# saidwivedi/TokenHMR

Hardware: AMD Instinct MI355X
Metric: crops_per_sec (higher is better)
Workload: dtype f32 (fp32 in / accumulate / out; the ViT GEMMs multiply each fp32 operand as three bf16 pieces on the bf16 MFMA pipe, six products per pair: `vit_gemm` split3; the fp32-MFMA mode is `exact_f32_mode`); 1 GPU; TokenHMR full path (ViT-H/16 + 6-layer token decoder + VQ lookup/decode + SMPL LBS), 256x256 crops, random-init weights; batch_per_gpu=64, global_batch=64, vit_depth=32, parallelism=dp1, allgather_outputs=False, vit_gemm=split3, ranks=1

## Files before the change

tokenhmr_amd/csrc/attention_b16.hip:

```cpp
#include "common.h"
#include "attention_device.h"
#include "gemm_split_device.h"

namespace {

constexpr int KB = 64;
constexpr int NBLK = NTOK / KB;
constexpr int KRS = 224;
constexpr int VRS = 160;
constexpr int KPL = KB * KRS;
constexpr int VPL = HD * VRS;
constexpr int K_IMG = 3 * KPL, V_IMG = 3 * VPL;
static_assert(2 * (K_IMG + V_IMG) <= 160 * 1024, "two workgroups per CU");
static_assert(V_IMG >= 4 * 16 * 480, "the split3 epilogue assembles 4 waves x 16 rows x 480 bytes in the dead V^T image");
constexpr float LOG2E_F = 1.44269504088896340736f;

typedef uint32_t u32x2v __attribute__((ext_vector_type(2)));

__device__ __forceinline__ bf16x8 pieces8(uint32_t a, uint32_t b, uint32_t c, uint32_t d) {
    return __builtin_bit_cast(bf16x8, u32x4{a, b, c, d});
}

template <int QT, bool SPLIT, int ABL = 0, int EARLY = 0, int OCC = 2>
__global__ __launch_bounds__(256, OCC) void vit_attention_b16_kernel(const float* __restrict__ qkv, float* __restrict__ out, int nitems) {
    constexpr int QB = 3 / QT;
    static_assert(QT == 1 || QT == 3, "192 queries = QB workgroups x 4 waves x QT tiles of 16");
    __shared__ __attribute__((aligned(16))) char smem[K_IMG + V_IMG];
    char* const kimg = smem;
    char* const vimg = smem + K_IMG;
    const int tid = threadIdx.x, lane = tid & 63;
    const int wave = __builtin_amdgcn_readfirstlane(tid >> 6);
    const int l15 = lane & 15, g = lane >> 4;
    const int xcd = blockIdx.x & 7, within = blockIdx.x >> 3, wpx = gridDim.x >> 3, per_xcd = nitems >> 3;
    int it = within;
    if (it >= per_xcd) return;
    struct Item { int crop, hcol, q0; };
    auto item_of = [&](int i) {
        const int lg = xcd * per_xcd + i, bh = lg / QB, qb = lg - bh * QB;
        return Item{bh / NH, (bh % NH) * HD, (qb * 4 + wave) * 16 * QT};
    };
    auto rsrc_of = [&](int crop) { return __builtin_amdgcn_make_buffer_rsrc(const_cast<float*>(qkv + (int64_t)crop * NTOK * QKV_LD), 0, NTOK * QKV_LD * 4, 0x00020000); };
    auto ld4 = [&](const Item& im, int uoff_floats, uint32_t off) {
        const u32x4 r = __builtin_amdgcn_raw_buffer_load_b128(rsrc_of(im.crop), off, uoff_floats * 4, 0);
        return f32x4{__uint_as_float(r[0]), __uint_as_float(r[1]), __uint_as_float(r[2]), __uint_as_float(r[3])};
    };
    auto ld1 = [&](const Item& im, int uoff_floats, uint32_t off) { return __uint_as_float(__builtin_amdgcn_raw_buffer_load_b32(rsrc_of(im.crop), off, uoff_floats * 4, 0)); };

    const int kkey = tid >> 2, kpart = tid & 3;
    const int vdg = (tid & 7) + 8 * ((tid >> 4) & 1), vkq = ((tid >> 5) & 3) | (((tid >> 3) & 1) << 2) | ((tid >> 7) << 3);
    const uint32_t koff = (uint32_t)(kkey * QKV_LD + kpart * 4) * 4u;
    const uint32_t voff = (uint32_t)(vkq * 4 * QKV_LD + vdg) * 4u;
    const uint32_t qoff = (uint32_t)(l15 * QKV_LD + g * 8) * 4u;
    char* const kdst = kimg + kkey * KRS + kpart * 8;
    char* const vdst = vimg + vdg * VRS + (((4 * (vkq >> 3) + (vkq & 3)) ^ ((vdg >> 2) & 1)) * 16) + 8 * ((vkq >> 2) & 1);
    f32x4 kr[5];
    float vr[5][4];
    auto load_k = [&](const Item& im, int blk) {
        const int ub = im.hcol + DIM + blk * KB * QKV_LD;
#pragma unroll
        for (int m = 0; m < 5; ++m) kr[m] = ld4(im, ub + m * 16, koff);
    };
    auto write_k = [&]() {
#pragma unroll
        for (int m = 0; m < 5; ++m) {
            uint32_t H[2], M[2], L[2];
            split3_pair(kr[m][0], kr[m][1], H[0], M[0], L[0]);
            split3_pair(kr[m][2], kr[m][3], H[1], M[1], L[1]);
            char* o = kdst + m * 32;
            *reinterpret_cast<u32x2v*>(o) = u32x2v{H[0], H[1]};
            *reinterpret_cast<u32x2v*>(o + KPL) = u32x2v{M[0], M[1]};
            *reinterpret_cast<u32x2v*>(o + 2 * KPL) = u32x2v{L[0], L[1]};
        }
    };
    auto load_v = [&](const Item& im, int blk) {
        const int ub = im.hcol + 2 * DIM + blk * KB * QKV_LD;
#pragma unroll
        for (int m = 0; m < 5; ++m)
#pragma unroll
            for (int r = 0; r < 4; ++r) vr[m][r] = ld1(im, ub + r * QKV_LD + m * 16, voff);
    };
    auto write_v = [&]() {
#pragma unroll
        for (int m = 0; m < 5; ++m) {
            uint32_t H[2], M[2], L[2];
            split3_pair(vr[m][0], vr[m][1], H[0], M[0], L[0]);
            split3_pair(vr[m][2], vr[m][3], H[1], M[1], L[1]);
            char* o = vdst + m * 16 * VRS;
            *reinterpret_cast<u32x2v*>(o) = u32x2v{H[0], H[1]};
            *reinterpret_cast<u32x2v*>(o + VPL) = u32x2v{M[0], M[1]};
            *reinterpret_cast<u32x2v*>(o + 2 * VPL) = u32x2v{L[0], L[1]};
        }
    };

    f32x4 qraw[QT][2];
    auto load_q = [&](const Item& im, int s) {
#pragma unroll
        for (int qt = 0; qt < QT; ++qt) {
            const int ub = im.hcol + (im.q0 + qt * 16) * QKV_LD + s * 32;
            if (s < 2 || g < 2) {
                qraw[qt][0] = ld4(im, ub, qoff);
                qraw[qt][1] = ld4(im, ub + 4, qoff);
            } else {
                qraw[qt][0] = f32x4{0.f, 0.f, 0.f, 0.f};
                qraw[qt][1] = f32x4{0.f, 0.f, 0.f, 0.f};
            }
        }
    };
    bf16x8 qf[QT][3];
    auto split_q = [&]() {
#pragma unroll
        for (int qt = 0; qt < QT; ++qt) {
            uint32_t H[4], M[4], L[4];
            split3_pair(qraw[qt][0][0], qraw[qt][0][1], H[0], M[0], L[0]);
            split3_pair(qraw[qt][0][2], qraw[qt][0][3], H[1], M[1], L[1]);
            split3_pair(qraw[qt][1][0], qraw[qt][1][1], H[2], M[2], L[2]);
            split3_pair(qraw[qt][1][2], qraw[qt][1][3], H[3], M[3], L[3]);
            qf[qt][0] = pieces8(H[0], H[1], H[2], H[3]);
            qf[qt][1] = pieces8(M[0], M[1], M[2], M[3]);
            qf[qt][2] = pieces8(L[0], L[1], L[2], L[3]);
        }
    };

    const char* const kfr = kimg + l15 * KRS + g * 16;
    const char* const vfr = vimg + l15 * VRS + ((g ^ ((l15 >> 2) & 1)) * 16);

    Item cur = item_of(it);
    load_k(cur, 0);
    load_q(cur, 0);
    for (int idx = tid; idx < 3 * KB * 2; idx += 256) {
        const int pl = idx / (2 * KB), rem = idx - pl * (2 * KB);
        *reinterpret_cast<u32x4*>(kimg + pl * KPL + (rem >> 1) * KRS + 160 + (rem & 1) * 16) = u32x4{0u, 0u, 0u, 0u};
    }
    write_k();
    __syncthreads();

#pragma unroll 1
    for (;;) {
        const bool has_next = it + wpx < per_xcd;
        const Item nxt = has_next ? item_of(it + wpx) : cur;
        f32x4 o[QT][5];
        float lsum[QT], cneg[QT];
#pragma unroll
        for (int qt = 0; qt < QT; ++qt) {
#pragma unroll
            for (int dt = 0; dt < 5; ++dt) o[qt][dt] = f32x4{0.f, 0.f, 0.f, 0.f};
            lsum[qt] = 0.f;
            cneg[qt] = 3.0e38f;
        }
#pragma unroll 1
        for (int blk = 0; blk < NBLK; ++blk) {
            const bool more = blk + 1 < NBLK;
            f32x4 s[QT][4];
#pragma unroll
            for (int qt = 0; qt < QT; ++qt)
#pragma unroll
                for (int kt = 0; kt < 4; ++kt) s[qt][kt] = f32x4{0.f, 0.f, 0.f, 0.f};
            bf16x8 kc[3], kn[3];
#pragma unroll
            for (int pc = 0; pc < 3; ++pc) kc[pc] = *reinterpret_cast<const bf16x8*>(kfr + pc * KPL);
#pragma unroll
            for (int st = 0; st < 3; ++st) {
                if constexpr (EARLY > 0 && (ABL & 2) == 0) {
                    if (st == EARLY - 1) {
                        load_v(cur, blk);
                        if (more) load_k(cur, blk + 1);
                        else if (has_next) load_k(nxt, 0);
                    }
                }
                if ((ABL & 4) == 0 || blk == 0) split_q();
                if (st + 1 < 3 && ((ABL & 1) == 0 || blk == 0)) load_q(cur, st + 1);
#pragma unroll
                for (int kt = 0; kt < 4; ++kt) {
                    const int nx = st * 4 + kt + 1;
                    if (nx < 12) {
#pragma unroll
                        for (int pc = 0; pc < 3; ++pc)
                            kn[pc] = *reinterpret_cast<const bf16x8*>(kfr + pc * KPL + (nx % 4) * 16 * KRS + (nx / 4) * 64);
                    }
                    __builtin_amdgcn_sched_barrier(0);
#pragma unroll
                    for (int p = 0; p < NPROD; ++p)
#pragma unroll
                        for (int qt = 0; qt < QT; ++qt)
                            s[qt][kt] = __builtin_amdgcn_mfma_f32_16x16x32_bf16(kc[piece_w(p)], qf[qt][piece_a(p)], s[qt][kt], 0, 0, 0);
                    __builtin_amdgcn_sched_barrier(0);
#pragma unroll
                    for (int pc = 0; pc < 3; ++pc) kc[pc] = kn[pc];
                }
            }
            if constexpr ((ABL & 2) == 0) {
                if constexpr (EARLY == 0) {
                    load_v(cur, blk);
                    if (more) load_k(cur, blk + 1);
                    else if (has_next) load_k(nxt, 0);
                }
            } else {
#pragma unroll
                for (int m = 0; m < 5; ++m) {
                    kr[m] = s[0][m & 3];
                    asm volatile("" : "+v"(kr[m]));
#pragma unroll
                    for (int r = 0; r < 4; ++r) {
                        vr[m][r] = s[0][(m + r) & 3][r];
                        asm volatile("" : "+v"(vr[m][r]));
                    }
                }
            }
            __syncthreads();
#pragma unroll
            for (int qt = 0; qt < QT; ++qt) {
                float m = s[qt][0][0];
#pragma unroll
                for (int kt = 0; kt < 4; ++kt)
#pragma unroll
                    for (int r = 0; r < 4; ++r) m = fmaxf(m, s[qt][kt][r]);
                m = fmaxf(m, __shfl_xor(m, 16, 64));
                m = fmaxf(m, __shfl_xor(m, 32, 64));
                const float c = fminf(-(m * LOG2E_F), cneg[qt]);
                const float alpha = __builtin_amdgcn_exp2f(c - cneg[qt]);
                cneg[qt] = c;
                lsum[qt] *= alpha;
#pragma unroll
                for (int dt = 0; dt < 5; ++dt) o[qt][dt] = o[qt][dt] * alpha;
                const f32x2 c2 = splat2(c), l2 = splat2(LOG2E_F);
                f32x2 sum2 = splat2(0.f);
#pragma unroll
                for (int kt = 0; kt < 4; ++kt)
#pragma unroll
                    for (int hh = 0; hh < 2; ++hh) {
                        const f32x2 t = __builtin_elementwise_fma(f32x2{s[qt][kt][2 * hh], s[qt][kt][2 * hh + 1]}, l2, c2);
                        const f32x2 e = f32x2{__builtin_amdgcn_exp2f(t.x), __builtin_amdgcn_exp2f(t.y)};
                        s[qt][kt][2 * hh] = e.x;
                        s[qt][kt][2 * hh + 1] = e.y;
                        sum2 += e;
                    }
                lsum[qt] += sum2.x + sum2.y;
            }
            write_v();
            if (more || has_next) write_k();
            __syncthreads();
            if constexpr ((ABL & 1) == 0) {
                if (more) load_q(cur, 0);
                else if (has_next) load_q(nxt, 0);
            } else if (!more && has_next) load_q(nxt, 0);
            bf16x8 vc[3], vn[3];
#pragma unroll
            for (int pc = 0; pc < 3; ++pc) vc[pc] = *reinterpret_cast<const bf16x8*>(vfr + pc * VPL);
#pragma unroll
            for (int st = 0; st < 2; ++st) {
                bf16x8 pf[QT][3];
#pragma unroll
                for (int qt = 0; qt < QT; ++qt) {
                    uint32_t H[4], M[4], L[4];
                    split3_pair(s[qt][2 * st][0], s[qt][2 * st][1], H[0], M[0], L[0]);
                    split3_pair(s[qt][2 * st][2], s[qt][2 * st][3], H[1], M[1], L[1]);
                    split3_pair(s[qt][2 * st + 1][0], s[qt][2 * st + 1][1], H[2], M[2], L[2]);
                    split3_pair(s[qt][2 * st + 1][2], s[qt][2 * st + 1][3], H[3], M[3], L[3]);
                    pf[qt][0] = pieces8(H[0], H[1], H[2], H[3]);
                    pf[qt][1] = pieces8(M[0], M[1], M[2], M[3]);
                    pf[qt][2] = pieces8(L[0], L[1], L[2], L[3]);
                }
#pragma unroll
                for (int dt = 0; dt < 5; ++dt) {
                    const int nx = st * 5 + dt + 1;
                    if (nx < 10) {
#pragma unroll
                        for (int pc = 0; pc < 3; ++pc)
                            vn[pc] = *reinterpret_cast<const bf16x8*>(vfr + pc * VPL + (nx % 5) * 16 * VRS + (nx / 5) * 64);
                    }
                    __builtin_amdgcn_sched_barrier(0);
#pragma unroll
                    for (int p = 0; p < NPROD; ++p)
#pragma unroll
                        for (int qt = 0; qt < QT; ++qt)
                            o[qt][dt] = __builtin_amdgcn_mfma_f32_16x16x32_bf16(vc[piece_w(p)], pf[qt][piece_a(p)], o[qt][dt], 0, 0, 0);
                    __builtin_amdgcn_sched_barrier(0);
#pragma unroll
                    for (int pc = 0; pc < 3; ++pc) vc[pc] = vn[pc];
                }
            }
        }

        float inv[QT];
#pragma unroll
        for (int qt = 0; qt < QT; ++qt) {
            float l = lsum[qt];
            l += __shfl_xor(l, 16, 64);
            l += __shfl_xor(l, 32, 64);
            inv[qt] = 1.0f / l;
        }
        if constexpr (SPLIT) {
            __syncthreads();
            char* const stg = vimg + wave * (16 * 480);
            char* const orow = reinterpret_cast<char*>(out) + ((int64_t)cur.crop * NTOK + cur.q0) * (DIM * 6) + cur.hcol * 6;
#pragma unroll
            for (int qt = 0; qt < QT; ++qt) {
                char* const srow = stg + l15 * 480;
#pragma unroll
                for (int pr = 0; pr < 2; ++pr) {
                    f32x4 x = o[qt][2 * pr] * inv[qt], y = o[qt][2 * pr + 1] * inv[qt];
#pragma unroll
                    for (int j = 0; j < 4; ++j) {
                        typedef uint32_t u32x2_t __attribute__((ext_vector_type(2)));
                        const u32x2_t sw = __builtin_amdgcn_permlane16_swap(__float_as_uint(x[j]), __float_as_uint(y[j]), false, false);
                        x[j] = __uint_as_float(sw.x);
                        y[j] = __uint_as_float(sw.y);
                    }
                    uint32_t H[4], M[4], L[4];
                    split3_pair(x[0], x[1], H[0], M[0], L[0]);
                    split3_pair(x[2], x[3], H[1], M[1], L[1]);
                    split3_pair(y[0], y[1], H[2], M[2], L[2]);
                    split3_pair(y[2], y[3], H[3], M[3], L[3]);
                    char* c = srow + ((2 * pr + (g & 1)) * 2 + (g >> 1)) * 48;
                    *reinterpret_cast<u32x4*>(c) = u32x4{H[0], H[1], H[2], H[3]};
                    *reinterpret_cast<u32x4*>(c + 16) = u32x4{M[0], M[1], M[2], M[3]};
                    *reinterpret_cast<u32x4*>(c + 32) = u32x4{L[0], L[1], L[2], L[3]};
                }
                {
                    const f32x4 v = o[qt][4] * inv[qt];
                    uint32_t H[2], M[2], L[2];
                    split3_pair(v[0], v[1], H[0], M[0], L[0]);
                    split3_pair(v[2], v[3], H[1], M[1], L[1]);
                    char* c = srow + (8 + (g >> 1)) * 48 + (g & 1) * 8;
                    *reinterpret_cast<u32x2v*>(c) = u32x2v{H[0], H[1]};
                    *reinterpret_cast<u32x2v*>(c + 16) = u32x2v{M[0], M[1]};
                    *reinterpret_cast<u32x2v*>(c + 32) = u32x2v{L[0], L[1]};
                }
#pragma unroll
                for (int i = 0; i < 8; ++i) {
                    const int c = i * 64 + lane;
                    if (i < 7 || lane < 32) {
                        const u32x4 v = *reinterpret_cast<const u32x4*>(stg + c * 16);
                        const int r = c / 30;
                        *reinterpret_cast<u32x4*>(orow + (int64_t)(qt * 16 + r) * (DIM * 6) + (c - r * 30) * 16) = v;
                    }
                }
            }
        } else {
            float* obase = out + (int64_t)cur.crop * NTOK * DIM + cur.hcol;
#pragma unroll
            for (int qt = 0; qt < QT; ++qt)
#pragma unroll
                for (int dt = 0; dt < 5; ++dt)
                    *reinterpret_cast<f32x4*>(obase + (int64_t)(cur.q0 + qt * 16 + l15) * DIM + dt * 16 + g * 4) = o[qt][dt] * inv[qt];
        }
        if (!has_next) break;
        cur = nxt;
        it += wpx;
    }
}

}

int launch_vit_attention_b16(const float* qkv, void* out, int B, bool out_split, int qt, hipStream_t s) {
    if (B <= 0 || (qt != 0 && qt != 1 && qt != 3)) return -1;
    if (qt == 0) qt = B <= 20 ? 1 : 3;
    float* o = reinterpret_cast<float*>(out);
    const int nitems = B * NH * (3 / qt);
    static_assert(NH % 8 == 0, "items per crop must divide by the XCD count");
    dim3 grid(nitems < 512 ? nitems : 512);
#ifdef THMR_EXPERIMENTS
    {
        const char* gk = thmr_knob("THMR_ATTN_GRID");
        const int gcap = gk ? atoi(gk) : 0;
        if (gcap >= 8 && (gcap % 8) == 0 && (unsigned)gcap < grid.x) grid = dim3(gcap);
        const char* ek = thmr_knob("THMR_ATTN_EARLY");
        const int early = ek ? atoi(ek) : 0;
        const char* ok = thmr_knob("THMR_ATTN_OCC");
        if (ok && ok[0] == '1' && qt == 3 && out_split) {
            if (grid.x > 256) grid = dim3(256);
            switch (early) {
                case 0: hipLaunchKernelGGL((vit_attention_b16_kernel<3, true, 0, 0, 1>), grid, dim3(256), 0, s, qkv, o, nitems); break;
                case 1: hipLaunchKernelGGL((vit_attention_b16_kernel<3, true, 0, 1, 1>), grid, dim3(256), 0, s, qkv, o, nitems); break;
                case 2: hipLaunchKernelGGL((vit_attention_b16_kernel<3, true, 0, 2, 1>), grid, dim3(256), 0, s, qkv, o, nitems); break;
                case 3: hipLaunchKernelGGL((vit_attention_b16_kernel<3, true, 0, 3, 1>), grid, dim3(256), 0, s, qkv, o, nitems); break;
                default: return -1;
            }
            return hipGetLastError() == hipSuccess ? 0 : -2;
        }
        if (early > 0 && qt == 3 && out_split) {
            switch (early) {
                case 1: hipLaunchKernelGGL((vit_attention_b16_kernel<3, true, 0, 1>), grid, dim3(256), 0, s, qkv, o, nitems); break;
                case 2: hipLaunchKernelGGL((vit_attention_b16_kernel<3, true, 0, 2>), grid, dim3(256), 0, s, qkv, o, nitems); break;
                case 3: hipLaunchKernelGGL((vit_attention_b16_kernel<3, true, 0, 3>), grid, dim3(256), 0, s, qkv, o, nitems); break;
                default: return -1;
            }
            return hipGetLastError() == hipSuccess ? 0 : -2;
        }
        const char* k = thmr_knob("THMR_ATTN_ABL");
        const int abl = k ? atoi(k) : 0;
        if (abl > 0 && qt == 3 && out_split) {
            switch (abl) {
                case 1: hipLaunchKernelGGL((vit_attention_b16_kernel<3, true, 1>), grid, dim3(256), 0, s, qkv, o, nitems); break;
                case 2: hipLaunchKernelGGL((vit_attention_b16_kernel<3, true, 2>), grid, dim3(256), 0, s, qkv, o, nitems); break;
                case 3: hipLaunchKernelGGL((vit_attention_b16_kernel<3, true, 3>), grid, dim3(256), 0, s, qkv, o, nitems); break;
                case 4: hipLaunchKernelGGL((vit_attention_b16_kernel<3, true, 4>), grid, dim3(256), 0, s, qkv, o, nitems); break;
                case 5: hipLaunchKernelGGL((vit_attention_b16_kernel<3, true, 5>), grid, dim3(256), 0, s, qkv, o, nitems); break;
                case 7: hipLaunchKernelGGL((vit_attention_b16_kernel<3, true, 7>), grid, dim3(256), 0, s, qkv, o, nitems); break;
                default: return -1;
            }
            return hipGetLastError() == hipSuccess ? 0 : -2;
        }
    }
#endif
    if (qt == 1) {
        if (out_split) hipLaunchKernelGGL((vit_attention_b16_kernel<1, true>), grid, dim3(256), 0, s, qkv, o, nitems);
        else hipLaunchKernelGGL((vit_attention_b16_kernel<1, false>), grid, dim3(256), 0, s, qkv, o, nitems);
    } else {
        if (out_split) hipLaunchKernelGGL((vit_attention_b16_kernel<3, true>), grid, dim3(256), 0, s, qkv, o, nitems);
        else hipLaunchKernelGGL((vit_attention_b16_kernel<3, false>), grid, dim3(256), 0, s, qkv, o, nitems);
    }
    return hipGetLastError() == hipSuccess ? 0 : -2;
}
```

Measured before the change: 855.9 crops/s.

## Keep Q pieces resident across key blocks and interleave softmax with attention MFMAs

Adds a RES mode that loads and splits all three Q slices once per item and keeps them in registers, so the per-block Q reload and re-split go away. Adds TILE modes that interleave one query tile's softmax and P splitting with the next tile's QK/PV MFMAs using sched_group_barrier placement. For B>=32 the default switches to resident Q with early K/V requests and occupancy 1 (grid capped at 256). This trades more registers and lower occupancy for less repeated work and better overlap.

```diff
diff --git a/tokenhmr_amd/csrc/attention_b16.hip b/tokenhmr_amd/csrc/attention_b16.hip
--- a/tokenhmr_amd/csrc/attention_b16.hip
+++ b/tokenhmr_amd/csrc/attention_b16.hip
@@ -21,10 +21,12 @@
     return __builtin_bit_cast(bf16x8, u32x4{a, b, c, d});
 }
 
-template <int QT, bool SPLIT, int ABL = 0, int EARLY = 0, int OCC = 2>
+template <int QT, bool SPLIT, int RES = 0, int EARLY = 0, int OCC = 2, int VPG = 2>
 __global__ __launch_bounds__(256, OCC) void vit_attention_b16_kernel(const float* __restrict__ qkv, float* __restrict__ out, int nitems) {
     constexpr int QB = 3 / QT;
     static_assert(QT == 1 || QT == 3, "192 queries = QB workgroups x 4 waves x QT tiles of 16");
+    constexpr bool TILE = RES == 2 || RES == 3;
+    static_assert(!TILE || QT == 3, "the per-tile interleave needs a wave with more than one query tile");
     __shared__ __attribute__((aligned(16))) char smem[K_IMG + V_IMG];
     char* const kimg = smem;
     char* const vimg = smem + K_IMG;
@@ -92,33 +94,38 @@
         }
     };
 
-    f32x4 qraw[QT][2];
-    auto load_q = [&](const Item& im, int s) {
+    constexpr int QS = RES ? 3 : 1;
+    f32x4 qraw[QS][QT][2];
+    auto load_q = [&](const Item& im, int s, int slot) {
 #pragma unroll
         for (int qt = 0; qt < QT; ++qt) {
             const int ub = im.hcol + (im.q0 + qt * 16) * QKV_LD + s * 32;
             if (s < 2 || g < 2) {
-                qraw[qt][0] = ld4(im, ub, qoff);
-                qraw[qt][1] = ld4(im, ub + 4, qoff);
+                qraw[slot][qt][0] = ld4(im, ub, qoff);
+                qraw[slot][qt][1] = ld4(im, ub + 4, qoff);
             } else {
-                qraw[qt][0] = f32x4{0.f, 0.f, 0.f, 0.f};
-                qraw[qt][1] = f32x4{0.f, 0.f, 0.f, 0.f};
-            }
-        }
-    };
-    bf16x8 qf[QT][3];
-    auto split_q = [&]() {
+                qraw[slot][qt][0] = f32x4{0.f, 0.f, 0.f, 0.f};
+                qraw[slot][qt][1] = f32x4{0.f, 0.f, 0.f, 0.f};
+            }
+        }
+    };
+    bf16x8 qf[QS][QT][3];
+    auto split_q = [&](int slot) {
 #pragma unroll
         for (int qt = 0; qt < QT; ++qt) {
             uint32_t H[4], M[4], L[4];
-            split3_pair(qraw[qt][0][0], qraw[qt][0][1], H[0], M[0], L[0]);
-            split3_pair(qraw[qt][0][2], qraw[qt][0][3], H[1], M[1], L[1]);
-            split3_pair(qraw[qt][1][0], qraw[qt][1][1], H[2], M[2], L[2]);
-            split3_pair(qraw[qt][1][2], qraw[qt][1][3], H[3], M[3], L[3]);
-            qf[qt][0] = pieces8(H[0], H[1], H[2], H[3]);
-            qf[qt][1] = pieces8(M[0], M[1], M[2], M[3]);
-            qf[qt][2] = pieces8(L[0], L[1], L[2], L[3]);
-        }
+            split3_pair(qraw[slot][qt][0][0], qraw[slot][qt][0][1], H[0], M[0], L[0]);
+            split3_pair(qraw[slot][qt][0][2], qraw[slot][qt][0][3], H[1], M[1], L[1]);
+            split3_pair(qraw[slot][qt][1][0], qraw[slot][qt][1][1], H[2], M[2], L[2]);
+            split3_pair(qraw[slot][qt][1][2], qraw[slot][qt][1][3], H[3], M[3], L[3]);
+            qf[slot][qt][0] = pieces8(H[0], H[1], H[2], H[3]);
+            qf[slot][qt][1] = pieces8(M[0], M[1], M[2], M[3]);
+            qf[slot][qt][2] = pieces8(L[0], L[1], L[2], L[3]);
+        }
+    };
+    auto load_q_item = [&](const Item& im) {
+#pragma unroll
+        for (int s = 0; s < 3; ++s) load_q(im, s, s);
     };
 
     const char* const kfr = kimg + l15 * KRS + g * 16;
@@ -126,7 +133,8 @@
 
     Item cur = item_of(it);
     load_k(cur, 0);
-    load_q(cur, 0);
+    if constexpr (RES) load_q_item(cur);
+    else load_q(cur, 0, 0);
     for (int idx = tid; idx < 3 * KB * 2; idx += 256) {
         const int pl = idx / (2 * KB), rem = idx - pl * (2 * KB);
         *reinterpret_cast<u32x4*>(kimg + pl * KPL + (rem >> 1) * KRS + 160 + (rem & 1) * 16) = u32x4{0u, 0u, 0u, 0u};
@@ -147,136 +155,255 @@
             lsum[qt] = 0.f;
             cneg[qt] = 3.0e38f;
         }
+        f32x4 s[QT][4];
+        float smax[QT], salpha[QT], sum0[QT], sum1[QT];
+        auto pin = [](auto&... v) {
+            if constexpr (RES >= 2) (..., [](auto& x) { asm volatile("" : "+v"(x)); }(v));
+        };
+        auto softmax_part = [&](int qt, int part) {
+            if (part == 0) {
+                float m = s[qt][0][0];
+#pragma unroll
+                for (int kt = 0; kt < 2; ++kt)
+#pragma unroll
+                    for (int r = 0; r < 4; ++r) m = fmaxf(m, s[qt][kt][r]);
+                smax[qt] = m;
+                pin(smax[qt]);
+            } else if (part == 1) {
+                float m = smax[qt];
+#pragma unroll
+                for (int kt = 2; kt < 4; ++kt)
+#pragma unroll
+                    for (int r = 0; r < 4; ++r) m = fmaxf(m, s[qt][kt][r]);
+                smax[qt] = m;
+                pin(smax[qt]);
+            } else if (part == 2) {
+                float m = smax[qt];
+                m = fmaxf(m, __shfl_xor(m, 16, 64));
+                m = fmaxf(m, __shfl_xor(m, 32, 64));
+                const float c = fminf(-(m * LOG2E_F), cneg[qt]);
+                salpha[qt] = __builtin_amdgcn_exp2f(c - cneg[qt]);
+                cneg[qt] = c;
+                sum0[qt] = 0.f;
+                sum1[qt] = 0.f;
+                pin(salpha[qt], cneg[qt]);
+            } else if (part == 3) {
+#pragma unroll
+                for (int dt = 0; dt < 5; ++dt)
+#pragma unroll
+                    for (int r = 0; r < 4; ++r) {
+                        o[qt][dt][r] = o[qt][dt][r] * salpha[qt];
+                        if constexpr (RES == 3) {
+                            if (r & 1) asm volatile("" : "+v"(o[qt][dt]));
+                        }
+                    }
+                pin(o[qt][0], o[qt][1], o[qt][2], o[qt][3], o[qt][4]);
+            } else {
+                const int kt = (part - 4) >> 1, hh = (part - 4) & 1;
+                const float e0 = __builtin_amdgcn_exp2f(__builtin_fmaf(s[qt][kt][2 * hh], LOG2E_F, cneg[qt]));
+                const float e1 = __builtin_amdgcn_exp2f(__builtin_fmaf(s[qt][kt][2 * hh + 1], LOG2E_F, cneg[qt]));
+                s[qt][kt][2 * hh] = e0;
+                s[qt][kt][2 * hh + 1] = e1;
+                sum0[qt] += e0;
+                sum1[qt] += e1;
+                if (part == 11) lsum[qt] = __builtin_fmaf(lsum[qt], salpha[qt], sum0[qt] + sum1[qt]);
+                pin(s[qt][kt], sum0[qt], sum1[qt], lsum[qt]);
+            }
+        };
+        uint32_t pw[QT][2][3][4];
+        auto psplit_part = [&](int qt, int part) {
+            const int st = part >> 2, j = part & 3;
+            const float x0 = s[qt][2 * st + (j >> 1)][2 * (j & 1)], x1 = s[qt][2 * st + (j >> 1)][2 * (j & 1) + 1];
+            if constexpr (RES == 3) {
+#pragma clang fp contract(off)
+                const uint32_t H = cvt_pk_bf16(x0, x1);
+                float r0 = x0 - __uint_as_float(H << 16), r1 = x1 - __uint_as_float(H & 0xffff0000u);
+                asm volatile("" : "+v"(r0));
+                const uint32_t M = cvt_pk_bf16(r0, r1);
+                r0 = r0 - __uint_as_float(M << 16);
+                asm volatile("" : "+v"(r0));
+                r1 = r1 - __uint_as_float(M & 0xffff0000u);
+                pw[qt][st][0][j] = H;
+                pw[qt][st][1][j] = M;
+                pw[qt][st][2][j] = cvt_pk_bf16(r0, r1);
+            } else split3_pair(x0, x1, pw[qt][st][0][j], pw[qt][st][1][j], pw[qt][st][2][j]);
+            pin(pw[qt][st][0][j], pw[qt][st][1][j], pw[qt][st][2][j]);
+        };
+        auto pfrag = [&](int qt, int st, int pc) { return pieces8(pw[qt][st][pc][0], pw[qt][st][pc][1], pw[qt][st][pc][2], pw[qt][st][pc][3]); };
+        auto place = [&]() {
+#pragma unroll
+            for (int p = 0; p < NPROD; ++p) {
+                __builtin_amdgcn_sched_group_barrier(0x8, 1, 0);
+                __builtin_amdgcn_sched_group_barrier(0x2, VPG, 0);
+            }
+        };
 #pragma unroll 1
         for (int blk = 0; blk < NBLK; ++blk) {
             const bool more = blk + 1 < NBLK;
-            f32x4 s[QT][4];
-#pragma unroll
-            for (int qt = 0; qt < QT; ++qt)
-#pragma unroll
-                for (int kt = 0; kt < 4; ++kt) s[qt][kt] = f32x4{0.f, 0.f, 0.f, 0.f};
+            auto request_kv = [&]() {
+                load_v(cur, blk);
+                if (more) load_k(cur, blk + 1);
+                else if (has_next) load_k(nxt, 0);
+            };
+            if constexpr (RES) {
+                if (blk == 0) {
+#pragma unroll
+                    for (int st = 0; st < 3; ++st) split_q(st);
+                }
+            }
             bf16x8 kc[3], kn[3];
 #pragma unroll
             for (int pc = 0; pc < 3; ++pc) kc[pc] = *reinterpret_cast<const bf16x8*>(kfr + pc * KPL);
-#pragma unroll
-            for (int st = 0; st < 3; ++st) {
-                if constexpr (EARLY > 0 && (ABL & 2) == 0) {
-                    if (st == EARLY - 1) {
-                        load_v(cur, blk);
-                        if (more) load_k(cur, blk + 1);
-                        else if (has_next) load_k(nxt, 0);
-                    }
-                }
-                if ((ABL & 4) == 0 || blk == 0) split_q();
-                if (st + 1 < 3 && ((ABL & 1) == 0 || blk == 0)) load_q(cur, st + 1);
-#pragma unroll
-                for (int kt = 0; kt < 4; ++kt) {
-                    const int nx = st * 4 + kt + 1;
-                    if (nx < 12) {
-#pragma unroll
-                        for (int pc = 0; pc < 3; ++pc)
-                            kn[pc] = *reinterpret_cast<const bf16x8*>(kfr + pc * KPL + (nx % 4) * 16 * KRS + (nx / 4) * 64);
-                    }
-                    __builtin_amdgcn_sched_barrier(0);
-#pragma unroll
-                    for (int p = 0; p < NPROD; ++p)
-#pragma unroll
-                        for (int qt = 0; qt < QT; ++qt)
-                            s[qt][kt] = __builtin_amdgcn_mfma_f32_16x16x32_bf16(kc[piece_w(p)], qf[qt][piece_a(p)], s[qt][kt], 0, 0, 0);
-                    __builtin_amdgcn_sched_barrier(0);
-#pragma unroll
-                    for (int pc = 0; pc < 3; ++pc) kc[pc] = kn[pc];
-                }
-            }
-            if constexpr ((ABL & 2) == 0) {
-                if constexpr (EARLY == 0) {
-                    load_v(cur, blk);
-                    if (more) load_k(cur, blk + 1);
-                    else if (has_next) load_k(nxt, 0);
+            if constexpr (!TILE) {
+#pragma unroll
+                for (int qt = 0; qt < QT; ++qt)
+#pragma unroll
+                    for (int kt = 0; kt < 4; ++kt) s[qt][kt] = f32x4{0.f, 0.f, 0.f, 0.f};
+#pragma unroll
+                for (int st = 0; st < 3; ++st) {
+                    if constexpr (EARLY > 0) {
+                        if (st == EARLY - 1) request_kv();
+                    }
+                    if constexpr (RES == 0) {
+                        split_q(0);
+                        if (st + 1 < 3) load_q(cur, st + 1, 0);
+                    }
+#pragma unroll
+                    for (int kt = 0; kt < 4; ++kt) {
+                        const int nx = st * 4 + kt + 1;
+                        if (nx < 12) {
+#pragma unroll
+                            for (int pc = 0; pc < 3; ++pc)
+                                kn[pc] = *reinterpret_cast<const bf16x8*>(kfr + pc * KPL + (nx % 4) * 16 * KRS + (nx / 4) * 64);
+                        }
+                        __builtin_amdgcn_sched_barrier(0);
+#pragma unroll
+                        for (int p = 0; p < NPROD; ++p)
+#pragma unroll
+                            for (int qt = 0; qt < QT; ++qt)
+                                s[qt][kt] = __builtin_amdgcn_mfma_f32_16x16x32_bf16(kc[piece_w(p)], qf[RES ? st : 0][qt][piece_a(p)], s[qt][kt], 0, 0, 0);
+                        __builtin_amdgcn_sched_barrier(0);
+#pragma unroll
+                        for (int pc = 0; pc < 3; ++pc) kc[pc] = kn[pc];
+                    }
                 }
             } else {
 #pragma unroll
-                for (int m = 0; m < 5; ++m) {
-                    kr[m] = s[0][m & 3];
-                    asm volatile("" : "+v"(kr[m]));
-#pragma unroll
-                    for (int r = 0; r < 4; ++r) {
-                        vr[m][r] = s[0][(m + r) & 3][r];
-                        asm volatile("" : "+v"(vr[m][r]));
-                    }
-                }
-            }
+                for (int qt = 0; qt < QT; ++qt) {
+                    if constexpr (EARLY > 0) {
+                        if (qt == EARLY - 1) request_kv();
+                    }
+#pragma unroll
+                    for (int gi = 0; gi < 12; ++gi) {
+                        const int st = gi >> 2, kt = gi & 3, nx = (qt * 12 + gi + 1) % 12;
+                        __builtin_amdgcn_sched_barrier(0);
+                        if (qt * 12 + gi + 1 < QT * 12) {
+#pragma unroll
+                            for (int pc = 0; pc < 3; ++pc)
+                                kn[pc] = *reinterpret_cast<const bf16x8*>(kfr + pc * KPL + (nx % 4) * 16 * KRS + (nx / 4) * 64);
+                        }
+                        if (st == 0) s[qt][kt] = f32x4{0.f, 0.f, 0.f, 0.f};
+                        if (qt > 0) softmax_part(qt - 1, gi);
+#pragma unroll
+                        for (int p = 0; p < NPROD; ++p)
+                            s[qt][kt] = __builtin_amdgcn_mfma_f32_16x16x32_bf16(kc[piece_w(p)], qf[st][qt][piece_a(p)], s[qt][kt], 0, 0, 0);
+                        if (qt > 0) place();
+                        __builtin_amdgcn_sched_barrier(0);
+#pragma unroll
+                        for (int pc = 0; pc < 3; ++pc) kc[pc] = kn[pc];
+                    }
+                }
+            }
+            if constexpr (EARLY == 0) request_kv();
             __syncthreads();
-#pragma unroll
-            for (int qt = 0; qt < QT; ++qt) {
-                float m = s[qt][0][0];
-#pragma unroll
-                for (int kt = 0; kt < 4; ++kt)
-#pragma unroll
-                    for (int r = 0; r < 4; ++r) m = fmaxf(m, s[qt][kt][r]);
-                m = fmaxf(m, __shfl_xor(m, 16, 64));
-                m = fmaxf(m, __shfl_xor(m, 32, 64));
-                const float c = fminf(-(m * LOG2E_F), cneg[qt]);
-                const float alpha = __builtin_amdgcn_exp2f(c - cneg[qt]);
-                cneg[qt] = c;
-                lsum[qt] *= alpha;
-#pragma unroll
-                for (int dt = 0; dt < 5; ++dt) o[qt][dt] = o[qt][dt] * alpha;
-                const f32x2 c2 = splat2(c), l2 = splat2(LOG2E_F);
-                f32x2 sum2 = splat2(0.f);
-#pragma unroll
-                for (int kt = 0; kt < 4; ++kt)
-#pragma unroll
-                    for (int hh = 0; hh < 2; ++hh) {
-                        const f32x2 t = __builtin_elementwise_fma(f32x2{s[qt][kt][2 * hh], s[qt][kt][2 * hh + 1]}, l2, c2);
-                        const f32x2 e = f32x2{__builtin_amdgcn_exp2f(t.x), __builtin_amdgcn_exp2f(t.y)};
-                        s[qt][kt][2 * hh] = e.x;
-                        s[qt][kt][2 * hh + 1] = e.y;
-                        sum2 += e;
-                    }
-                lsum[qt] += sum2.x + sum2.y;
+            if constexpr (!TILE) {
+#pragma unroll
+                for (int qt = 0; qt < QT; ++qt)
+#pragma unroll
+                    for (int part = 0; part < 12; ++part) softmax_part(qt, part);
+            } else {
+#pragma unroll
+                for (int part = 0; part < 8; ++part) psplit_part(0, part);
             }
             write_v();
             if (more || has_next) write_k();
             __syncthreads();
-            if constexpr ((ABL & 1) == 0) {
-                if (more) load_q(cur, 0);
-                else if (has_next) load_q(nxt, 0);
-            } else if (!more && has_next) load_q(nxt, 0);
+            if constexpr (RES == 0) {
+                if (more) load_q(cur, 0, 0);
+                else if (has_next) load_q(nxt, 0, 0);
+            } else {
+                if (!more && has_next) load_q_item(nxt);
+            }
             bf16x8 vc[3], vn[3];
 #pragma unroll
             for (int pc = 0; pc < 3; ++pc) vc[pc] = *reinterpret_cast<const bf16x8*>(vfr + pc * VPL);
-#pragma unroll
-            for (int st = 0; st < 2; ++st) {
-                bf16x8 pf[QT][3];
+            if constexpr (!TILE) {
+#pragma unroll
+                for (int st = 0; st < 2; ++st) {
+#pragma unroll
+                    for (int qt = 0; qt < QT; ++qt)
+#pragma unroll
+                        for (int j = 0; j < 4; ++j)
+                            if (RES != 4 || st == 0) psplit_part(qt, 4 * st + j);
+#pragma unroll
+                    for (int dt = 0; dt < 5; ++dt) {
+                        const int nx = st * 5 + dt + 1;
+                        if constexpr (RES == 4) {
+                            __builtin_amdgcn_sched_barrier(0);
+                            if (st == 0) {
+#pragma unroll
+                                for (int u = dt * (4 * QT) / 5; u < (dt + 1) * (4 * QT) / 5; ++u) psplit_part(u >> 2, 4 + (u & 3));
+                            }
+                        }
+                        if (nx < 10) {
+#pragma unroll
+                            for (int pc = 0; pc < 3; ++pc)
+                                vn[pc] = *reinterpret_cast<const bf16x8*>(vfr + pc * VPL + (nx % 5) * 16 * VRS + (nx / 5) * 64);
+                        }
+                        if constexpr (RES != 4) __builtin_amdgcn_sched_barrier(0);
+#pragma unroll
+                        for (int p = 0; p < NPROD; ++p)
+#pragma unroll
+                            for (int qt = 0; qt < QT; ++qt)
+                                o[qt][dt] = __builtin_amdgcn_mfma_f32_16x16x32_bf16(vc[piece_w(p)], pfrag(qt, st, piece_a(p)), o[qt][dt], 0, 0, 0);
+                        if constexpr (RES == 4) {
+                            if (st == 0) {
+#pragma unroll
+                                for (int qt = 0; qt < QT; ++qt) place();
+                            }
+                        }
+                        __builtin_amdgcn_sched_barrier(0);
+#pragma unroll
+                        for (int pc = 0; pc < 3; ++pc) vc[pc] = vn[pc];
+                    }
+                }
+            } else {
 #pragma unroll
                 for (int qt = 0; qt < QT; ++qt) {
-                    uint32_t H[4], M[4], L[4];
-                    split3_pair(s[qt][2 * st][0], s[qt][2 * st][1], H[0], M[0], L[0]);
-                    split3_pair(s[qt][2 * st][2], s[qt][2 * st][3], H[1], M[1], L[1]);
-                    split3_pair(s[qt][2 * st + 1][0], s[qt][2 * st + 1][1], H[2], M[2], L[2]);
-                    split3_pair(s[qt][2 * st + 1][2], s[qt][2 * st + 1][3], H[3], M[3], L[3]);
-                    pf[qt][0] = pieces8(H[0], H[1], H[2], H[3]);
-                    pf[qt][1] = pieces8(M[0], M[1], M[2], M[3]);
-                    pf[qt][2] = pieces8(L[0], L[1], L[2], L[3]);
-                }
-#pragma unroll
-                for (int dt = 0; dt < 5; ++dt) {
-                    const int nx = st * 5 + dt + 1;
-                    if (nx < 10) {
-#pragma unroll
-                        for (int pc = 0; pc < 3; ++pc)
-                            vn[pc] = *reinterpret_cast<const bf16x8*>(vfr + pc * VPL + (nx % 5) * 16 * VRS + (nx / 5) * 64);
-                    }
-                    __builtin_amdgcn_sched_barrier(0);
-#pragma unroll
-                    for (int p = 0; p < NPROD; ++p)
-#pragma unroll
-                        for (int qt = 0; qt < QT; ++qt)
-                            o[qt][dt] = __builtin_amdgcn_mfma_f32_16x16x32_bf16(vc[piece_w(p)], pf[qt][piece_a(p)], o[qt][dt], 0, 0, 0);
-                    __builtin_amdgcn_sched_barrier(0);
-#pragma unroll
-                    for (int pc = 0; pc < 3; ++pc) vc[pc] = vn[pc];
+#pragma unroll
+                    for (int gi = 0; gi < 10; ++gi) {
+                        const int st = gi / 5, dt = gi % 5, nx = (qt * 10 + gi + 1) % 10;
+                        __builtin_amdgcn_sched_barrier(0);
+                        if (qt * 10 + gi + 1 < QT * 10) {
+#pragma unroll
+                            for (int pc = 0; pc < 3; ++pc)
+                                vn[pc] = *reinterpret_cast<const bf16x8*>(vfr + pc * VPL + (nx % 5) * 16 * VRS + (nx / 5) * 64);
+                        }
+                        if (qt == 0) {
+                            if (gi < 2) {
+                                softmax_part(QT - 1, 2 * gi);
+                                softmax_part(QT - 1, 2 * gi + 1);
+                            } else softmax_part(QT - 1, gi + 2);
+                        }
+                        if (qt + 1 < QT && (qt > 0 ? gi < 8 : gi >= 2)) psplit_part(qt + 1, qt > 0 ? gi : gi - 2);
+#pragma unroll
+                        for (int p = 0; p < NPROD; ++p)
+                            o[qt][dt] = __builtin_amdgcn_mfma_f32_16x16x32_bf16(vc[piece_w(p)], pfrag(qt, st, piece_a(p)), o[qt][dt], 0, 0, 0);
+                        if (qt + 1 < QT) place();
+                        __builtin_amdgcn_sched_barrier(0);
+#pragma unroll
+                        for (int pc = 0; pc < 3; ++pc) vc[pc] = vn[pc];
+                    }
                 }
             }
         }
@@ -350,6 +477,23 @@
     }
 }
 
+constexpr int P3_MIN_B = 32;
+constexpr int P3_RES = 1, P3_EARLY = 1, P3_OCC = 1, P3_VPG = 2;
+constexpr int P1_RES = 1;
+
+template <int QT, bool SPLIT, int RES, int EARLY, int OCC, int VPG>
+int launch_body(const float* qkv, float* o, int nitems, hipStream_t s) {
+    const int cap = OCC == 1 ? 256 : 512;
+    dim3 grid(nitems < cap ? nitems : cap);
+#ifdef THMR_EXPERIMENTS
+    const char* gk = thmr_knob("THMR_ATTN_GRID");
+    const int gcap = gk ? atoi(gk) : 0;
+    if (gcap >= 8 && (gcap % 8) == 0 && (unsigned)gcap < grid.x) grid = dim3(gcap);
+#endif
+    hipLaunchKernelGGL((vit_attention_b16_kernel<QT, SPLIT, RES, EARLY, OCC, VPG>), grid, dim3(256), 0, s, qkv, o, nitems);
+    return hipGetLastError() == hipSuccess ? 0 : -2;
+}
+
 }
 
 int launch_vit_attention_b16(const float* qkv, void* out, int B, bool out_split, int qt, hipStream_t s) {
@@ -358,57 +502,35 @@
     float* o = reinterpret_cast<float*>(out);
     const int nitems = B * NH * (3 / qt);
     static_assert(NH % 8 == 0, "items per crop must divide by the XCD count");
-    dim3 grid(nitems < 512 ? nitems : 512);
 #ifdef THMR_EXPERIMENTS
     {
-        const char* gk = thmr_knob("THMR_ATTN_GRID");
-        const int gcap = gk ? atoi(gk) : 0;
-        if (gcap >= 8 && (gcap % 8) == 0 && (unsigned)gcap < grid.x) grid = dim3(gcap);
-        const char* ek = thmr_knob("THMR_ATTN_EARLY");
-        const int early = ek ? atoi(ek) : 0;
-        const char* ok = thmr_knob("THMR_ATTN_OCC");
-        if (ok && ok[0] == '1' && qt == 3 && out_split) {
-            if (grid.x > 256) grid = dim3(256);
-            switch (early) {
-                case 0: hipLaunchKernelGGL((vit_attention_b16_kernel<3, true, 0, 0, 1>), grid, dim3(256), 0, s, qkv, o, nitems); break;
-                case 1: hipLaunchKernelGGL((vit_attention_b16_kernel<3, true, 0, 1, 1>), grid, dim3(256), 0, s, qkv, o, nitems); break;
-                case 2: hipLaunchKernelGGL((vit_attention_b16_kernel<3, true, 0, 2, 1>), grid, dim3(256), 0, s, qkv, o, nitems); break;
-                case 3: hipLaunchKernelGGL((vit_attention_b16_kernel<3, true, 0, 3, 1>), grid, dim3(256), 0, s, qkv, o, nitems); break;
+        const char* ak = thmr_knob("THMR_ATTN_ARM");
+        const int arm = ak ? atoi(ak) : 0;
+        if (arm > 0 && out_split) {
+            if (qt == 3) switch (arm) {
+                case 22: return launch_body<3, true, 0, 0, 2, 2>(qkv, o, nitems, s);
+                case 12: return launch_body<3, true, 0, 0, 1, 2>(qkv, o, nitems, s);
+                case 1012: return launch_body<3, true, 1, 0, 1, 2>(qkv, o, nitems, s);
+                case 1112: return launch_body<3, true, 1, 1, 1, 2>(qkv, o, nitems, s);
+                case 2012: return launch_body<3, true, 2, 0, 1, 2>(qkv, o, nitems, s);
+                case 2112: return launch_body<3, true, 2, 1, 1, 2>(qkv, o, nitems, s);
+                case 2113: return launch_body<3, true, 2, 1, 1, 3>(qkv, o, nitems, s);
+                case 2212: return launch_body<3, true, 2, 2, 1, 2>(qkv, o, nitems, s);
+                case 3112: return launch_body<3, true, 3, 1, 1, 2>(qkv, o, nitems, s);
+                case 4112: return launch_body<3, true, 4, 1, 1, 2>(qkv, o, nitems, s);
+                case 4111: return launch_body<3, true, 4, 1, 1, 1>(qkv, o, nitems, s);
                 default: return -1;
             }
-            return hipGetLastError() == hipSuccess ? 0 : -2;
-        }
-        if (early > 0 && qt == 3 && out_split) {
-            switch (early) {
-                case 1: hipLaunchKernelGGL((vit_attention_b16_kernel<3, true, 0, 1>), grid, dim3(256), 0, s, qkv, o, nitems); break;
-                case 2: hipLaunchKernelGGL((vit_attention_b16_kernel<3, true, 0, 2>), grid, dim3(256), 0, s, qkv, o, nitems); break;
-                case 3: hipLaunchKernelGGL((vit_attention_b16_kernel<3, true, 0, 3>), grid, dim3(256), 0, s, qkv, o, nitems); break;
+            switch (arm) {
+                case 22: return launch_body<1, true, 0, 0, 2, 2>(qkv, o, nitems, s);
+                case 1022: return launch_body<1, true, 1, 0, 2, 2>(qkv, o, nitems, s);
                 default: return -1;
             }
-            return hipGetLastError() == hipSuccess ? 0 : -2;
-        }
-        const char* k = thmr_knob("THMR_ATTN_ABL");
-        const int abl = k ? atoi(k) : 0;
-        if (abl > 0 && qt == 3 && out_split) {
-            switch (abl) {
-                case 1: hipLaunchKernelGGL((vit_attention_b16_kernel<3, true, 1>), grid, dim3(256), 0, s, qkv, o, nitems); break;
-                case 2: hipLaunchKernelGGL((vit_attention_b16_kernel<3, true, 2>), grid, dim3(256), 0, s, qkv, o, nitems); break;
-                case 3: hipLaunchKernelGGL((vit_attention_b16_kernel<3, true, 3>), grid, dim3(256), 0, s, qkv, o, nitems); break;
-                case 4: hipLaunchKernelGGL((vit_attention_b16_kernel<3, true, 4>), grid, dim3(256), 0, s, qkv, o, nitems); break;
-                case 5: hipLaunchKernelGGL((vit_attention_b16_kernel<3, true, 5>), grid, dim3(256), 0, s, qkv, o, nitems); break;
-                case 7: hipLaunchKernelGGL((vit_attention_b16_kernel<3, true, 7>), grid, dim3(256), 0, s, qkv, o, nitems); break;
-                default: return -1;
-            }
-            return hipGetLastError() == hipSuccess ? 0 : -2;
         }
     }
 #endif
-    if (qt == 1) {
-        if (out_split) hipLaunchKernelGGL((vit_attention_b16_kernel<1, true>), grid, dim3(256), 0, s, qkv, o, nitems);
-        else hipLaunchKernelGGL((vit_attention_b16_kernel<1, false>), grid, dim3(256), 0, s, qkv, o, nitems);
-    } else {
-        if (out_split) hipLaunchKernelGGL((vit_attention_b16_kernel<3, true>), grid, dim3(256), 0, s, qkv, o, nitems);
-        else hipLaunchKernelGGL((vit_attention_b16_kernel<3, false>), grid, dim3(256), 0, s, qkv, o, nitems);
-    }
-    return hipGetLastError() == hipSuccess ? 0 : -2;
+    if (qt == 1) return out_split ? launch_body<1, true, P1_RES, 0, 2, 2>(qkv, o, nitems, s) : launch_body<1, false, P1_RES, 0, 2, 2>(qkv, o, nitems, s);
+    if (B < P3_MIN_B) return out_split ? launch_body<3, true, 0, 0, 2, 2>(qkv, o, nitems, s) : launch_body<3, false, 0, 0, 2, 2>(qkv, o, nitems, s);
+    return out_split ? launch_body<3, true, P3_RES, P3_EARLY, P3_OCC, P3_VPG>(qkv, o, nitems, s)
+                     : launch_body<3, false, P3_RES, P3_EARLY, P3_OCC, P3_VPG>(qkv, o, nitems, s);
 }
```

Result: no change. 856.9 crops/s (median of 6 runs) (+0.1%).
